# CESSProject/DeOSS

Hardware: AMD Instinct MI355X
Metric: device-resident GiB/s hashed to Merkle root; 1/2/4/8 MI355X scaling (higher is better)
Workload: dtype u32; 1 GPU; BASELINE configs[1]: 1 object of 8 GiB (8589934592 B) in 1 chunk-range shard(s) of 8 GiB, chunk 33554432 B (256 leaves); object_bytes=8589934592, chunk=33554432, leaves=256, parallelism=single GPU

## Files before the change

deoss_amd/csrc/merkle_kernels.hpp:

```cpp
#pragma once
#include "sha256_gfx950.hpp"

namespace dm {

constexpr int kBlock = 256;
constexpr int kLeafFuseMax = 8;
constexpr int kReduceTile = 512;

struct LeafArgs {
    const uint8_t* base;
    uint64_t pitch;
    uint64_t leaf_len;
    uint64_t last_len;
    const uint64_t* addrs;
    const uint64_t* lens;
    uint64_t nleaves;
    uint64_t byte_off;
    uint64_t byte_end;
    uint32_t* state;
    uint8_t* digests;
    uint8_t* level_out;
    uint32_t fuse_levels;
};

// ... 108 lines not shown
        compress(st, w);
    } else {
        compress(st, w);
#pragma unroll
        for (int k = 0; k < 14; k++) w[k] = 0;
        w[14] = (uint32_t)(bits >> 32);
        w[15] = (uint32_t)bits;
        compress(st, w);
    }
}

__device__ __forceinline__ uint32_t lds_reduce(uint32_t (*a)[8], uint32_t (*b)[8], uint32_t cnt,
                                               uint32_t levels, uint32_t (**res)[8]) {
    const uint32_t t = threadIdx.x;
    for (uint32_t l = 0; l < levels; l++) {
        const uint32_t next = (cnt + 1) >> 1;
        if (t < next) {
            uint32_t L[8], R[8], o[8];
            const uint32_t ri = (2 * t + 1 < cnt) ? 2 * t + 1 : cnt - 1;
#pragma unroll
            for (int k = 0; k < 8; k++) { L[k] = a[2 * t][k]; R[k] = a[ri][k]; }
            node_hash(L, R, o);
#pragma unroll
            for (int k = 0; k < 8; k++) b[t][k] = o[k];
        }
        __syncthreads();
        uint32_t (*tmp)[8] = a; a = b; b = tmp;
        cnt = next;
    }
    *res = a;
    return cnt;
}

struct LeafView {
    const uint8_t* p;
    uint64_t len;
    uint64_t have;
    uint64_t nb;
    bool fin;
    bool active;
};

template <bool TABLE>
__device__ __forceinline__ LeafView leaf_view(const LeafArgs& a, uint64_t i) {
    LeafView v{};
    v.active = i < a.nleaves;
    if (!v.active) {
        v.p = a.base;
        return v;
    }
    if constexpr (TABLE) {
        v.p = reinterpret_cast<const uint8_t*>(a.addrs[i]);
        v.len = a.lens[i];
    } else {
        v.p = a.base + i * a.pitch;
        v.len = (i + 1 == a.nleaves) ? a.last_len : a.leaf_len;
    }
    const uint64_t b0 = a.byte_off;
    const uint64_t end = v.len < a.byte_end ? v.len : a.byte_end;
    v.have = end > b0 ? end - b0 : 0;
    v.fin = (b0 < v.len && v.len <= a.byte_end) || (v.len == 0 && b0 == 0);
    v.nb = v.have / 64;
    return v;
}

__device__ __forceinline__ void load_or_init_state(const LeafArgs& a, uint64_t i, uint32_t (&st)[8]) {
    if (a.state != nullptr && a.byte_off != 0) {
#pragma unroll
        for (int k = 0; k < 8; k++) st[k] = a.state[i * 8 + k];
    } else {
        init_state(st);
    }
}

template <bool ALIGNED>
__device__ __forceinline__ void leaf_epilogue(const LeafArgs& a, uint64_t i, const LeafView& v, uint32_t (&st)[8]) {
    if (v.fin) {
        absorb_tail<ALIGNED>(st, v.p + 64 * v.nb, (uint32_t)(v.have - 64 * v.nb), v.len);
        if (a.digests != nullptr) store_digest(a.digests + 32 * i, st);
    } else if (a.state != nullptr && v.have != 0) {
#pragma unroll
        for (int k = 0; k < 8; k++) a.state[i * 8 + k] = st[k];
    }
}

__device__ __forceinline__ uint64_t wave_max_u64(uint64_t x) {
#pragma unroll
    for (int o = 32; o > 0; o >>= 1) {
        const uint64_t y = __shfl_xor(x, o, 64);
        x = y > x ? y : x;
    }
    return x;
}

template <bool TABLE, bool ALIGNED>
__global__ __launch_bounds__(kBlock) void leaf_kernel(LeafArgs a) {
    __shared__ uint32_t lds_a[kBlock][8];
    __shared__ uint32_t lds_b[kBlock / 2][8];
    const uint64_t i = (uint64_t)blockIdx.x * kBlock + threadIdx.x;
    const LeafView v = leaf_view<TABLE>(a, i);
    const bool active = v.active;
    uint32_t st[8];
    if (active) {
        load_or_init_state(a, i, st);
        absorb_blocks<ALIGNED>(st, v.p, v.nb);
        leaf_epilogue<ALIGNED>(a, i, v, st);
    }
    if (a.fuse_levels == 0) return;
    const uint64_t first = (uint64_t)blockIdx.x * kBlock;
    const uint32_t cnt = (uint32_t)((a.nleaves - first) < kBlock ? (a.nleaves - first) : kBlock);
    if (active) {
#pragma unroll
        for (int k = 0; k < 8; k++) lds_a[threadIdx.x][k] = st[k];
    }
    __syncthreads();
    uint32_t (*res)[8];
    const uint32_t out_cnt = lds_reduce(lds_a, lds_b, cnt, a.fuse_levels, &res);
    if (threadIdx.x < out_cnt) {
        uint32_t v[8];
#pragma unroll
        for (int k = 0; k < 8; k++) v[k] = res[threadIdx.x][k];
        const uint64_t o = (uint64_t)blockIdx.x * (kBlock >> a.fuse_levels) + threadIdx.x;
        store_digest(a.level_out + 32 * o, v);
    }
}

constexpr int kLatLeaves = 64;
constexpr int kLatThreads = 128;
constexpr int kLatRing = 2;
constexpr int kLatFuseMax = 6;

__device__ __forceinline__ void rounds_from_kw(uint32_t (&st)[8], const uint4 (*kw)[kLatLeaves], uint32_t lane) {
    uint32_t a = st[0], b = st[1], c = st[2], d = st[3], e = st[4], f = st[5], g = st[6], h = st[7];
    uint4 x = kw[0][lane], y = kw[1][lane];
#pragma unroll
    for (int q = 0; q < 16; q += 2) {
        uint4 nx = x, ny = y;
        if (q + 2 < 16) {
            nx = kw[q + 2][lane];
            ny = kw[q + 3][lane];
        }
        DM_SHA_ROUND(a, b, c, d, e, f, g, h, x.x);
        DM_SHA_ROUND(h, a, b, c, d, e, f, g, x.y);
        DM_SHA_ROUND(g, h, a, b, c, d, e, f, x.z);
        DM_SHA_ROUND(f, g, h, a, b, c, d, e, x.w);
        DM_SHA_ROUND(e, f, g, h, a, b, c, d, y.x);
        DM_SHA_ROUND(d, e, f, g, h, a, b, c, y.y);
        DM_SHA_ROUND(c, d, e, f, g, h, a, b, y.z);
        DM_SHA_ROUND(b, c, d, e, f, g, h, a, y.w);
        x = nx;
        y = ny;
    }
    st[0] += a; st[1] += b; st[2] += c; st[3] += d;
    st[4] += e; st[5] += f; st[6] += g; st[7] += h;
}

__device__ __forceinline__ void schedule_to_lds(uint32_t (&w)[16], uint4 (*kw)[kLatLeaves], uint32_t lane) {
#pragma unroll
    for (int q = 0; q < 16; q++) {
        uint32_t v[4];
#pragma unroll
        for (int j = 0; j < 4; j++) {
            const int t = 4 * q + j;
            uint32_t wt;
            if (t < 16) {
                wt = w[t];
// ... 109 lines not shown
    const uint64_t first = (uint64_t)blockIdx.x * kPairLeaves;
    const uint64_t i = first + c;
    const LeafView v = leaf_view<TABLE>(a, i);
    const uint64_t NB = wave_max_u64(v.nb);
    if (producer) {
        Blk cur;
        if (v.nb > 0 && !lane_b) cur = load_block<ALIGNED>(v.p);
        for (uint64_t b = 0; b < NB; b++) {
            if (b < v.nb) {
                uint32_t w[16];
                block_words(cur, w);
                if (b + 1 < v.nb && !lane_b) cur = load_block<ALIGNED>(v.p + 64 * (b + 1));
                uint4 (*kw)[kLatLeaves] = ring[b % kLatRing];
#pragma unroll
                for (int q = 0; q < 16; q++) {
                    uint32_t u[4];
#pragma unroll
                    for (int j = 0; j < 4; j++) {
                        const int t = 4 * q + j;
                        uint32_t wt;
                        if (t < 16) {
                            wt = w[t];
                        } else {
                            wt = ssig1(w[(t - 2) & 15]) + w[(t - 7) & 15] + ssig0(w[(t - 15) & 15]) + w[t & 15];
                            w[t & 15] = wt;
                        }
                        u[j] = lane_b ? 0u : kSha256K[t] + wt;
                    }
                    kw[q][lane] = make_uint4(u[0], u[1], u[2], u[3]);
                }
            }
            __syncthreads();
        }
        __syncthreads();
    } else {
        const uint32_t sh1 = lane_b ? 2 : 6, sh2 = lane_b ? 13 : 11, sh3 = lane_b ? 22 : 25;
        const uint32_t msk = lane_b ? 0u : ~0u;
        uint32_t st0[8];
        if (v.active) load_or_init_state(a, i, st0);
        else init_state(st0);
        uint32_t x[4];
#pragma unroll
        for (int k = 0; k < 4; k++) x[k] = lane_b ? st0[k] : st0[4 + k];
        __syncthreads();
        for (uint64_t b = 0; b < NB; b++) {
            if (b < v.nb) pair_rounds_from_kw(x, ring[b % kLatRing], lane, sh1, sh2, sh3, msk, lane_b);
            __syncthreads();
        }
        uint32_t st[8];
#pragma unroll
        for (int k = 0; k < 4; k++) {
            const uint32_t other = dpp_swap_pairs(x[k]);
            st[k] = lane_b ? x[k] : other;
            st[4 + k] = lane_b ? other : x[k];
        }
        if (v.active && !lane_b) {
            leaf_epilogue<ALIGNED>(a, i, v, st);
#pragma unroll
            for (int k = 0; k < 8; k++) lds_a[c][k] = st[k];
        }
    }
    if (a.fuse_levels == 0) return;
    __syncthreads();
    const uint32_t cnt = (uint32_t)((a.nleaves - first) < kPairLeaves ? (a.nleaves - first) : kPairLeaves);
    uint32_t (*res)[8];
    const uint32_t out_cnt = lds_reduce(lds_a, lds_b, cnt, a.fuse_levels, &res);
    if (threadIdx.x < out_cnt) {
        uint32_t o8[8];
#pragma unroll
        for (int k = 0; k < 8; k++) o8[k] = res[threadIdx.x][k];
        const uint64_t o = (uint64_t)blockIdx.x * (kPairLeaves >> a.fuse_levels) + threadIdx.x;
        store_digest(a.level_out + 32 * o, o8);
    }
}

constexpr int kQuadLeaves = 8;
constexpr int kQuadBlocks = 8;
constexpr int kQuadFuseMax = 3;
constexpr int kQuadRow = kQuadLeaves;
constexpr size_t kQuadLdsBytes = sizeof(uint4) * kLatRing * 16 * kQuadBlocks * kQuadRow + 4 * 8 * kQuadLeaves +
                                 4 * 8 * (kQuadLeaves / 2);
static_assert(4 * kQuadLdsBytes <= (160u << 10), "four compact K1Q workgroups must fit a CU's LDS");

#ifndef DM_QS_DEEP3
#define DM_QS_DEEP3 0
#endif
#if DM_QS_DEEP3
#define DM_QS_HEAD(X4, X5, X6)                                                                   \
    "v_alignbit_b32 %[r], %[" X4 "], %[" X4 "], %[sh]\n\t"                                      \
    "v_alignbit_b32 %[s], %[" X4 "], %[" X4 "], %[sh2]\n\t"                                     \
    "v_alignbit_b32 %[t], %[" X4 "], %[" X4 "], %[sh3]\n\t"                                     \
    "v_bitop3_b32 %[f], %[" X4 "], %[" X5 "], %[msk] bitop3:0x1e\n\t"                          \
    "v_bitop3_b32 %[f], %[f], %[" X6 "], %[" X5 "] bitop3:0xca\n\t"
#define DM_QS_SIGMA "v_bitop3_b32 %[s], %[r], %[s], %[t] bitop3:0x96\n\t"
#else
#define DM_QS_HEAD(X4, X5, X6)                                                                   \
    "v_alignbit_b32 %[r], %[" X4 "], %[" X4 "], %[sh]\n\t"                                      \
    "v_bitop3_b32 %[f], %[" X4 "], %[" X5 "], %[msk] bitop3:0x1e\n\t"                          \
    "v_bitop3_b32 %[f], %[f], %[" X6 "], %[" X5 "] bitop3:0xca\n\t"                             \
    "v_xor_b32_dpp %[s], %[r], %[r] quad_perm:[1,2,0,3] row_mask:0xf bank_mask:0xf\n\t"
#define DM_QS_SIGMA "v_xor_b32_dpp %[s], %[r], %[s] quad_perm:[2,0,1,3] row_mask:0xf bank_mask:0xf\n\t"
#endif
#define DM_QS_STEP_Q(X4, X5, X6, X7, H, HN, VN, QP)                                             \
    DM_QS_HEAD(X4, X5, X6)                                                                       \
    "v_sub_u32_dpp %[" X6 "], %[" VN "], %[" X6 "] quad_perm:" QP " row_mask:0xf bank_mask:0x3\n\t" \
    DM_QS_SIGMA                                                                                  \
    "v_sub_u32_dpp %[" HN "], %[" X4 "], %[" X6 "] row_ror:8 row_mask:0xf bank_mask:0xf\n\t"    \
    "v_add3_u32 %[" X7 "], %[s], %[f], %[" H "]\n\t"
#define DM_QS_STEP(X4, X5, X6, X7, H, HN, VN) DM_QS_STEP_Q(X4, X5, X6, X7, H, HN, VN, "[0,1,2,3]")
#define DM_QS_STEP_A(X4, X5, X6, X7, H, HN)                                                     \
    DM_QS_HEAD(X4, X5, X6)                                                                       \
    DM_QS_SIGMA                                                                                  \
    "v_sub_u32_dpp %[" HN "], %[" X4 "], %[" X6 "] row_ror:8 row_mask:0xf bank_mask:0xf\n\t"    \
    "v_add3_u32 %[" X7 "], %[s], %[f], %[" H "]\n\t"
#define DM_QS_STEP_END(X4, X5, X6, X7, H)                                                       \
    DM_QS_HEAD(X4, X5, X6)                                                                       \
    DM_QS_SIGMA                                                                                  \
    "v_add3_u32 %[" X7 "], %[s], %[f], %[" H "]\n\t"
#define DM_QS_STEPS4V(V0, V1, V2, V3)                                                          \
    DM_QS_STEP("a", "b", "c", "d", "h", "g", V0) DM_QS_STEP("d", "a", "b", "c", "g", "h", V1)   \
    DM_QS_STEP("c", "d", "a", "b", "h", "g", V2) DM_QS_STEP("b", "c", "d", "a", "g", "h", V3)
#define DM_QS_ALIGN ".p2align 3\n\t"
#define DM_QS_ALIGN_MIS ".p2align 3\n\t.if %[mis]\n\ts_nop 0\n\t.endif\n\t"
#define DM_QS_PROLOGUE(V) DM_QS_PROLOGUE_AT(V, DM_QS_ALIGN, "[0,1,2,3]")
#define DM_QS_PROLOGUE_AT(V, ALIGN, QP)                                                           \
    "s_nop 1\n\t" ALIGN                                                                          \
    "v_sub_u32_dpp %[d], %[" V "], %[d] quad_perm:" QP " row_mask:0xf bank_mask:0x3\n\t"         \
    "v_sub_u32_dpp %[h], %[b], %[d] row_ror:8 row_mask:0xf bank_mask:0xf\n\t"
#define DM_QS_RESTORE_A(P, X) "v_mov_b32_dpp %[" P "], %[" X "] quad_perm:[0,1,2,3] row_mask:0xf bank_mask:0xc\n\t"
#define DM_QS_GROUP0(V0, V1, V2, V3)                                                             \
    DM_QS_STEP("a", "b", "c", "d", "h", "g", V0) DM_QS_RESTORE_A("d", "x3")                      \
    DM_QS_STEP("d", "a", "b", "c", "g", "h", V1) DM_QS_RESTORE_A("c", "x2")                      \
    DM_QS_STEP("c", "d", "a", "b", "h", "g", V2) DM_QS_STEP("b", "c", "d", "a", "g", "h", V3)
#define DM_QS_FF(X, P, BANKS) "v_add_u32_dpp %[" X "], %[" P "], %[" X "] quad_perm:[0,1,2,3] row_mask:0xf bank_mask:" BANKS "\n\t"
#define DM_QS_TAIL(V0, V1, V2)                                                                   \
    DM_QS_STEP("a", "b", "c", "d", "h", "g", V0) DM_QS_STEP("d", "a", "b", "c", "g", "h", V1)   \
    DM_QS_STEP("c", "d", "a", "b", "h", "g", V2) DM_QS_STEP_A("b", "c", "d", "a", "g", "h")      \
    DM_QS_FF("x3", "d", "0x3") DM_QS_FF("x2", "c", "0x3") DM_QS_FF("x1", "b", "0x3")             \
    DM_QS_FF("x0", "a", "0x3")                                                                   \
    DM_QS_STEP_A("a", "b", "c", "d", "h", "g") DM_QS_STEP_END("d", "a", "b", "c", "g")           \
    DM_QS_FF("x0", "a", "0xc") DM_QS_FF("x1", "b", "0xc") DM_QS_FF("x3", "d", "0xc")             \
    DM_QS_FF("x2", "c", "0xc")
#define DM_QS_STEPS4Q(V0, Q0, V1, Q1, V2, Q2, V3, Q3)                                          \
    DM_QS_STEP_Q("a", "b", "c", "d", "h", "g", V0, Q0) DM_QS_STEP_Q("d", "a", "b", "c", "g", "h", V1, Q1) \
    DM_QS_STEP_Q("c", "d", "a", "b", "h", "g", V2, Q2) DM_QS_STEP_Q("b", "c", "d", "a", "g", "h", V3, Q3)
#define DM_QS_GROUP0Q(V0, Q0, V1, Q1, V2, Q2, V3, Q3)                                          \
    DM_QS_STEP_Q("a", "b", "c", "d", "h", "g", V0, Q0) DM_QS_RESTORE_A("d", "x3")              \
    DM_QS_STEP_Q("d", "a", "b", "c", "g", "h", V1, Q1) DM_QS_RESTORE_A("c", "x2")              \
    DM_QS_STEP_Q("c", "d", "a", "b", "h", "g", V2, Q2) DM_QS_STEP_Q("b", "c", "d", "a", "g", "h", V3, Q3)
#define DM_QS_TAILQ(V0, Q0, V1, Q1, V2, Q2)                                                     \
    DM_QS_STEP_Q("a", "b", "c", "d", "h", "g", V0, Q0) DM_QS_STEP_Q("d", "a", "b", "c", "g", "h", V1, Q1) \
    DM_QS_STEP_Q("c", "d", "a", "b", "h", "g", V2, Q2) DM_QS_STEP_A("b", "c", "d", "a", "g", "h") \
    DM_QS_FF("x3", "d", "0x3") DM_QS_FF("x2", "c", "0x3") DM_QS_FF("x1", "b", "0x3")             \
    DM_QS_FF("x0", "a", "0x3")                                                                   \
    DM_QS_STEP_A("a", "b", "c", "d", "h", "g") DM_QS_STEP_END("d", "a", "b", "c", "g")           \
    DM_QS_FF("x0", "a", "0xc") DM_QS_FF("x1", "b", "0xc") DM_QS_FF("x3", "d", "0xc")             \
    DM_QS_FF("x2", "c", "0xc")
#if DM_QS_DEEP3
#define DM_QS_XOUT , [t] "=&v"(t_)
#define DM_QS_XIN , [sh2] "v"(sh.y), [sh3] "v"(sh.z)
#else
#define DM_QS_XOUT
#define DM_QS_XIN
#endif
#define DM_QS_OUT                                                                                \
    : [a] "+v"(p0), [b] "+v"(p1), [c] "+v"(p2), [d] "+v"(p3), [h] "+v"(h), [g] "+v"(g),           \
      [x0] "+v"(x[0]), [x1] "+v"(x[1]), [x2] "+v"(x[2]), [x3] "+v"(x[3]), [r] "=&v"(r_),          \
      [f] "=&v"(f_), [s] "=&v"(s_) DM_QS_XOUT
#define DM_QS_OPS DM_QS_OUT : [sh] "v"(sh.x), [msk] "v"(msk), [v0] "v"(v0), [v1] "v"(v1), [v2] "v"(v2), [v3] "v"(v3) DM_QS_XIN

template <class KW>
__device__ __forceinline__ void quad_block_skewed(uint32_t (&x)[4], KW kw, uint3 sh, uint32_t msk) {
    uint32_t p0 = x[0], p1 = x[1], p2 = x[2], p3 = x[3], h = 0, g = 0, r_, f_, s_, t_;
    (void)t_;
    uint4 q = kw(0), nq = kw(1);
    {
        const uint32_t v0 = q.x, v1 = 0, v2 = 0, v3 = 0;
        asm volatile(DM_QS_PROLOGUE("v0") DM_QS_OPS);
    }
#pragma unroll
    for (int grp = 0; grp < 16; grp++) {
        const uint4 nnq = grp + 2 < 16 ? kw(grp + 2) : nq;
        const uint32_t v0 = q.y, v1 = q.z, v2 = q.w, v3 = nq.x;
        if (grp == 0) {
            asm volatile(DM_QS_ALIGN DM_QS_GROUP0("v0", "v1", "v2", "v3") DM_QS_OPS);
        } else if (grp < 15) {
            asm volatile(DM_QS_ALIGN DM_QS_STEPS4V("v0", "v1", "v2", "v3") DM_QS_OPS);
        } else {
            asm volatile(DM_QS_ALIGN DM_QS_TAIL("v0", "v1", "v2") DM_QS_OPS);
        }
        q = nq;
        nq = nnq;
    }
}

constexpr int kLgkmWait0 = 0xC07F;

template <bool MIS>
__device__ __forceinline__ void quad_block_regs(uint32_t (&x)[4], const uint4 (&K)[4], uint3 sh, uint32_t msk) {
    uint32_t p0 = x[0], p1 = x[1], p2 = x[2], p3 = x[3], h, g, r_, f_, s_, t_;
    (void)t_;
    asm volatile(DM_QS_PROLOGUE_AT("q00", DM_QS_ALIGN_MIS, "[0,0,0,0]")
                 DM_QS_GROUP0Q("q01", "[0,0,0,0]", "q02", "[0,0,0,0]", "q03", "[0,0,0,0]", "q00", "[1,1,1,1]")
                 DM_QS_STEPS4Q("q01", "[1,1,1,1]", "q02", "[1,1,1,1]", "q03", "[1,1,1,1]", "q00", "[2,2,2,2]")
                 DM_QS_STEPS4Q("q01", "[2,2,2,2]", "q02", "[2,2,2,2]", "q03", "[2,2,2,2]", "q00", "[3,3,3,3]")
                 DM_QS_STEPS4Q("q01", "[3,3,3,3]", "q02", "[3,3,3,3]", "q03", "[3,3,3,3]", "q10", "[0,0,0,0]")
                 DM_QS_STEPS4Q("q11", "[0,0,0,0]", "q12", "[0,0,0,0]", "q13", "[0,0,0,0]", "q10", "[1,1,1,1]")
                 DM_QS_STEPS4Q("q11", "[1,1,1,1]", "q12", "[1,1,1,1]", "q13", "[1,1,1,1]", "q10", "[2,2,2,2]")
                 DM_QS_STEPS4Q("q11", "[2,2,2,2]", "q12", "[2,2,2,2]", "q13", "[2,2,2,2]", "q10", "[3,3,3,3]")
                 DM_QS_STEPS4Q("q11", "[3,3,3,3]", "q12", "[3,3,3,3]", "q13", "[3,3,3,3]", "q20", "[0,0,0,0]")
                 DM_QS_STEPS4Q("q21", "[0,0,0,0]", "q22", "[0,0,0,0]", "q23", "[0,0,0,0]", "q20", "[1,1,1,1]")
                 DM_QS_STEPS4Q("q21", "[1,1,1,1]", "q22", "[1,1,1,1]", "q23", "[1,1,1,1]", "q20", "[2,2,2,2]")
                 DM_QS_STEPS4Q("q21", "[2,2,2,2]", "q22", "[2,2,2,2]", "q23", "[2,2,2,2]", "q20", "[3,3,3,3]")
                 DM_QS_STEPS4Q("q21", "[3,3,3,3]", "q22", "[3,3,3,3]", "q23", "[3,3,3,3]", "q30", "[0,0,0,0]")
                 DM_QS_STEPS4Q("q31", "[0,0,0,0]", "q32", "[0,0,0,0]", "q33", "[0,0,0,0]", "q30", "[1,1,1,1]")
                 DM_QS_STEPS4Q("q31", "[1,1,1,1]", "q32", "[1,1,1,1]", "q33", "[1,1,1,1]", "q30", "[2,2,2,2]")
                 DM_QS_STEPS4Q("q31", "[2,2,2,2]", "q32", "[2,2,2,2]", "q33", "[2,2,2,2]", "q30", "[3,3,3,3]")
                 DM_QS_TAILQ("q31", "[3,3,3,3]", "q32", "[3,3,3,3]", "q33", "[3,3,3,3]")
                 : [a] "+v"(p0), [b] "+v"(p1), [c] "+v"(p2), [d] "+v"(p3), [h] "=&v"(h), [g] "=&v"(g),
                   [x0] "+v"(x[0]), [x1] "+v"(x[1]), [x2] "+v"(x[2]), [x3] "+v"(x[3]), [r] "=&v"(r_),
                   [f] "=&v"(f_), [s] "=&v"(s_) DM_QS_XOUT
                 : [mis] "i"(MIS ? 1 : 0), [sh] "v"(sh.x), [msk] "v"(msk),
                   [q00] "v"(K[0].x), [q01] "v"(K[0].y), [q02] "v"(K[0].z), [q03] "v"(K[0].w),
                   [q10] "v"(K[1].x), [q11] "v"(K[1].y), [q12] "v"(K[1].z), [q13] "v"(K[1].w),
                   [q20] "v"(K[2].x), [q21] "v"(K[2].y), [q22] "v"(K[2].z), [q23] "v"(K[2].w),
                   [q30] "v"(K[3].x), [q31] "v"(K[3].y), [q32] "v"(K[3].z), [q33] "v"(K[3].w) DM_QS_XIN);
}

template <int G, int ROW, bool MIS>
__device__ __forceinline__ void quad_stage_regs(uint32_t (&x)[4], const uint4* kw, uint3 sh, uint32_t msk) {
    uint4 A[4], B[4];
#pragma unroll
    for (int t = 0; t < 4; t++) A[t] = kw[4 * t * G];
#pragma unroll
    for (int k = 0; k < kQuadBlocks; k += 2) {
        __builtin_amdgcn_s_waitcnt(kLgkmWait0);
#pragma unroll
        for (int t = 0; t < 4; t++) B[t] = kw[(k + 1) * ROW + 4 * t * G];
        quad_block_regs<MIS>(x, A, sh, msk);
        __builtin_amdgcn_s_waitcnt(kLgkmWait0);
        if (k + 2 < kQuadBlocks) {
#pragma unroll
            for (int t = 0; t < 4; t++) A[t] = kw[(k + 2) * ROW + 4 * t * G];
        }
        quad_block_regs<MIS>(x, B, sh, msk);
    }
}

template <bool TABLE, bool ALIGNED, bool COMPACT>
__global__ __launch_bounds__(kLatThreads) void leaf_kernel_quad(LeafArgs a) {
    constexpr int ROW = COMPACT ? kQuadRow : kQuadLeaves;
    constexpr int G = kQuadBlocks * ROW;
    __shared__ uint4 ring[COMPACT ? 1 : 2][kLatRing][16][G];
    __shared__ uint32_t lds_a[kQuadLeaves][8];
    __shared__ uint32_t lds_b[kQuadLeaves / 2][8];
    const uint32_t lane = threadIdx.x & 63;
    const bool producer = __builtin_amdgcn_readfirstlane(threadIdx.x) < 64;
    const uint32_t c = lane >> 3;
    const uint32_t j = lane & 7;
    const uint64_t first = (uint64_t)blockIdx.x * kQuadLeaves;
    const uint64_t i = first + c;
    const LeafView v = leaf_view<TABLE>(a, i);
    const uint64_t NB = wave_max_u64(v.nb);
    const uint64_t NI = (NB + kQuadBlocks - 1) / kQuadBlocks;
    if (producer) {
        Blk cur;
        if (j < v.nb) cur = load_block<ALIGNED>(v.p + 64 * j);
        for (uint64_t it = 0; it < NI; it++) {
            const uint64_t b = it * kQuadBlocks + j;
            if (b < v.nb) {
                uint32_t w[16];
                block_words(cur, w);
                if (b + kQuadBlocks < v.nb) cur = load_block<ALIGNED>(v.p + 64 * (b + kQuadBlocks));
                uint4* kw = &ring[0][it % kLatRing][0][j * ROW + c];
#pragma unroll
                for (int q = 0; q < 16; q++) {
                    uint32_t u[4];
#pragma unroll
                    for (int k = 0; k < 4; k++) {
                        const int t = 4 * q + k;
                        uint32_t wt;
                        if (t < 16) {
                            wt = w[t];
                        } else {
                            wt = ssig1(w[(t - 2) & 15]) + w[(t - 7) & 15] + ssig0(w[(t - 15) & 15]) + w[t & 15];
                            w[t & 15] = wt;
                        }
                        u[k] = 0u - (kSha256K[t] + wt);
                    }
                    kw[q * G] = make_uint4(u[0], u[1], u[2], u[3]);
                }
            }
            __syncthreads();
        }
        __syncthreads();
    } else {
        __builtin_amdgcn_s_setprio(1);
        const uint32_t cq = 2 * (lane >> 4) + ((lane >> 2) & 1);
        const bool role_a = (lane >> 3) & 1;
        const uint32_t p = lane & 3;
        const uint64_t iq = first + cq;
        const LeafView vq = leaf_view<TABLE>(a, iq);
#if DM_QS_DEEP3
        const uint3 sh = role_a ? make_uint3(2, 13, 22) : make_uint3(6, 11, 25);
#else
        const uint3 sh = make_uint3(role_a ? (p == 0 ? 2 : p == 1 ? 13 : 22) : (p == 0 ? 6 : p == 1 ? 11 : 25), 0, 0);
#endif
        const uint32_t msk = role_a ? 0u : ~0u;
        uint32_t st0[8];
        if (vq.active) load_or_init_state(a, iq, st0);
        else init_state(st0);
        uint32_t x[4];
#pragma unroll
        for (int k = 0; k < 4; k++) x[k] = role_a ? st0[(k + 2) & 3] : st0[4 + k];
        const uint4* col = &ring[0][0][0][cq];
        __syncthreads();
        uint32_t xf[4];
#pragma unroll
        for (int k = 0; k < 4; k++) xf[k] = x[k];
        auto partial = [&](uint64_t it) {
            const uint64_t b0 = it * kQuadBlocks;
            return __any(vq.active && vq.nb > b0 && vq.nb < b0 + kQuadBlocks);
        };
        for (uint64_t it = 0; it < NI;) {
            for (; it < NI && !partial(it); it++) {
                quad_stage_regs<G, ROW, COMPACT>(x, col + (it % kLatRing) * 16 * G + p * G, sh, msk);
                if (vq.nb > it * kQuadBlocks) {
#pragma unroll
                    for (int k = 0; k < 4; k++) xf[k] = x[k];
                }
                __syncthreads();
            }
            if (it == NI) break;
            const uint4* kw = col + (it % kLatRing) * 16 * G;
            const uint64_t b0 = it * kQuadBlocks;
            for (uint32_t k = 0; k < kQuadBlocks; k++) {
                const uint4* kb = kw + k * ROW;
                if (b0 + k < vq.nb)
                    quad_block_skewed(x, [kb](int g) { return kb[g * G]; }, sh, msk);
            }
            if (vq.nb > b0) {
#pragma unroll
                for (int k = 0; k < 4; k++) xf[k] = x[k];
            }
            __syncthreads();
            it++;
        }
        uint32_t st[8];
#pragma unroll
        for (int k = 0; k < 4; k++) {
            st[k] = __shfl(xf[(k + 2) & 3], (int)(lane + 8), 64);
            st[4 + k] = xf[k];
        }
        if (vq.active && !role_a && p == 0) {
            leaf_epilogue<ALIGNED>(a, iq, vq, st);
#pragma unroll
            for (int k = 0; k < 8; k++) lds_a[cq][k] = st[k];
        }
    }
    if (a.fuse_levels == 0) return;
    __syncthreads();
    const uint32_t cnt = (uint32_t)((a.nleaves - first) < kQuadLeaves ? (a.nleaves - first) : kQuadLeaves);
    uint32_t (*res)[8];
    const uint32_t out_cnt = lds_reduce(lds_a, lds_b, cnt, a.fuse_levels, &res);
    if (threadIdx.x < out_cnt) {
        uint32_t o8[8];
#pragma unroll
        for (int k = 0; k < 8; k++) o8[k] = res[threadIdx.x][k];
        const uint64_t o = (uint64_t)blockIdx.x * (kQuadLeaves >> a.fuse_levels) + threadIdx.x;
        store_digest(a.level_out + 32 * o, o8);
    }
}

__global__ __launch_bounds__(kLatThreads) void quad_shape_primer(int x) {
    extern __shared__ uint4 dyn[];
    if (x == 12345) dyn[threadIdx.x] = make_uint4(1, 1, 1, 1);
}

__global__ __launch_bounds__(kBlock) void reduce_kernel(const uint8_t* in, uint64_t m, uint32_t levels,
                                                         uint8_t* out) {
    __shared__ uint32_t lds_a[kBlock][8];
    __shared__ uint32_t lds_b[kBlock / 2][8];
    const uint64_t base = (uint64_t)blockIdx.x * kReduceTile;
    const uint32_t cnt = (uint32_t)((m - base) < kReduceTile ? (m - base) : kReduceTile);
    const uint32_t t = threadIdx.x;
    const uint32_t next = (cnt + 1) >> 1;
    if (t < next) {
        uint32_t L[8], R[8], o[8];
        const uint32_t ri = (2 * t + 1 < cnt) ? 2 * t + 1 : cnt - 1;
        load_digest(in + 32 * (base + 2 * t), L);
        load_digest(in + 32 * (base + ri), R);
        node_hash(L, R, o);
#pragma unroll
        for (int k = 0; k < 8; k++) lds_a[t][k] = o[k];
    }
    __syncthreads();
    uint32_t (*res)[8];
    const uint32_t out_cnt = lds_reduce(lds_a, lds_b, next, levels - 1, &res);
    if (t < out_cnt) {
        uint32_t v[8];
#pragma unroll
        for (int k = 0; k < 8; k++) v[k] = res[t][k];
        store_digest(out + 32 * ((uint64_t)blockIdx.x * (kReduceTile >> levels) + t), v);
    }
}

__global__ __launch_bounds__(kBlock) void batch_root_kernel(const uint8_t* leaves, const uint64_t* leaf_first,
                                                             const uint32_t* obj_ids, uint8_t* roots) {
    __shared__ uint32_t lds_a[kBlock][8];
    __shared__ uint32_t lds_b[kBlock / 2][8];
    const uint32_t o = obj_ids[blockIdx.x];
    const uint64_t base = leaf_first[o];
    const uint32_t cnt = (uint32_t)(leaf_first[o + 1] - base);
    const uint32_t t = threadIdx.x;
    const uint32_t next = (cnt + 1) >> 1;
    if (t < next) {
        uint32_t L[8], R[8], h[8];
        const uint32_t ri = (2 * t + 1 < cnt) ? 2 * t + 1 : cnt - 1;
        load_digest(leaves + 32 * (base + 2 * t), L);
        load_digest(leaves + 32 * (base + ri), R);
        node_hash(L, R, h);
#pragma unroll
// ... 68 lines not shown
```

deoss_amd/isa.py:

```python
from __future__ import annotations

import json
import os
import re
import subprocess
import tempfile

HERE = os.path.dirname(os.path.abspath(__file__))
COUNTS = os.path.join(HERE, "isa_counts.json")
SLOT_WEIGHTS = {"v_alignbit_b32": 2.0, "v_add3_u32": 2.0, "v_xad_u32": 2.0}
KERNELS = {
    "wide": ("_ZN2dm11leaf_kernelILb0ELb1EEEvNS_8LeafArgsE", (1, 0)),
    "latency": ("_ZN2dm15leaf_kernel_latILb0ELb1EEEvNS_8LeafArgsE", (1, 1)),
    "pair": ("_ZN2dm16leaf_kernel_pairILb0ELb1EEEvNS_8LeafArgsE", (2, 2)),
    "quad": ("_ZN2dm16leaf_kernel_quadILb0ELb1ELb0EEEvNS_8LeafArgsE", (8, 1)),
}
K1_SYMBOL = KERNELS["wide"][0]


def _function_body(asm: str, sym: str) -> list:
    lines = asm.splitlines()
    start = None
    for i, ln in enumerate(lines):
        if ln.startswith(sym + ":"):
            start = i
            break
    if start is None:
        raise ValueError(f"{sym} not found in assembly")
    body = []
    for ln in lines[start + 1:]:
        if ln.startswith(".Lfunc_end") or re.match(r"^\s*\.size\s+" + re.escape(sym), ln):
            break
        body.append(ln)
    return body


def _loops(body: list):
    labels, insts = {}, []
    skip = []
    for ln in body:
        s = ln.strip()
        m = re.match(r"^\.if\s+(\S+)", s)
        if m:
            skip.append(m.group(1) == "0")
            continue
        if s.startswith(".endif"):
            if skip:
                skip.pop()
            continue
        if any(skip):
            continue
        m = re.match(r"^(\.LBB[0-9_]+):", s)
        if m:
            labels[m.group(1)] = len(insts)
            continue
        if not s or s.startswith(";") or s.startswith("."):
            continue
        insts.append(s.split(";")[0].strip())
    for i, ins in enumerate(insts):
        m = re.match(r"^s_c?branch\w*\s+(\.LBB[0-9_]+)", ins)
        if m and m.group(1) in labels and labels[m.group(1)] <= i:
            yield insts[labels[m.group(1)]:i + 1]


def _summary(loop: list, per: int) -> dict:
    valu = [x for x in loop if x.startswith("v_")]
    hist = {}
    for x in valu:
        op = x.split()[0]
        hist[op] = hist.get(op, 0) + 1
    slots = sum(SLOT_WEIGHTS.get(x.split()[0], 1.0) for x in valu)
    return {"valu": round(len(valu) / per, 1), "valu_slots": round(slots / per, 1),
            "blocks_per_iteration": per, "salu": sum(1 for x in loop if x.startswith("s_")),
            "lds": sum(1 for x in loop if x.startswith("ds_")),
            "vmem": sum(1 for x in loop if x.startswith(("global_", "buffer_", "flat_"))),
            "total": len(loop), "valu_histogram": dict(sorted(hist.items(), key=lambda kv: -kv[1]))}


def _smallest(loops, pred):
    best = None
    for lp in loops:
        if pred(lp) and (best is None or len(lp) < len(best)):
            best = lp
    return best


def analyse(asm: str, sym: str = K1_SYMBOL) -> dict:
    loops = [l for l in _loops(_function_body(asm, sym))
             if sum(x.startswith("global_load_dwordx4") for x in l) >= 4]
    if not loops:
        raise ValueError("no block loop found")
    lp = max(loops, key=len)
    loads = sum(x.startswith("global_load_dwordx4") for x in lp)
    return _summary(lp, max(1, loads // 4))


def analyse_split(asm: str, sym: str) -> dict:
    loops = list(_loops(_function_body(asm, sym)))
    stage = _smallest(loops, lambda l: sum(x.startswith("v_add3_u32") for x in l) >= 8 * 66
                      and sum(x.startswith("ds_read_b128") for x in l) >= 32)
    if stage is not None:
        prod = _smallest(loops, lambda l: sum(x.startswith("ds_write_b128") for x in l) >= 16)
        if prod is None:
            raise ValueError(f"{sym}: producer loop not found")
        return {"consumer": _summary(stage, 8), "producer": _summary(prod, 1)}
    cons = _smallest(loops, lambda l: sum(x.startswith("ds_read_b128") for x in l) >= 16)
    prod = _smallest(loops, lambda l: sum(x.startswith("ds_write_b128") for x in l) >= 16)
    if cons is None or prod is None:
        raise ValueError(f"{sym}: consumer/producer loop not found")
    return {"consumer": _summary(cons, 1), "producer": _summary(prod, 1)}


def generate(write: bool = True) -> dict:
    from . import build as b
    with tempfile.TemporaryDirectory() as td:
        out = os.path.join(td, "lib.so")
        cmd = b.hipcc_cmd(out, extra=("-save-temps",))
        subprocess.run(cmd, check=True, cwd=td, capture_output=True)
        asm_files = [f for f in os.listdir(td) if f.endswith(".s") and "gfx950" in f]
        asm = open(os.path.join(td, asm_files[0])).read()
    res = {}
    for name, (sym, lanes) in KERNELS.items():
        if name == "wide":
            d = analyse(asm, sym)
            d["lane_slots_per_leaf_block"] = d["valu_slots"]
        else:
            d = analyse_split(asm, sym)
            d["lane_slots_per_leaf_block"] = (d["consumer"]["valu_slots"] * lanes[0] +
                                              d["producer"]["valu_slots"] * lanes[1])
            d["consumer_valu_per_block"] = d["consumer"]["valu"]
        d["kernel"] = sym
        d["lanes_per_leaf_block"] = {"consumer": lanes[0], "producer": lanes[1]}
        res[name] = d
    res["per"] = "one 64-byte block of one leaf"
    if write:
        with open(COUNTS, "w") as f:
            json.dump(res, f, indent=1)
    return res


def kernel_counts(kind: str = "wide"):
    try:
        with open(COUNTS) as f:
            d = json.load(f)[kind]
    except (OSError, KeyError, ValueError):
        return None, None
    ops = d["valu"] if kind == "wide" else d["consumer_valu_per_block"]
    return ops, d["lane_slots_per_leaf_block"]


def valu_per_block():
    return kernel_counts("wide")


def chain_instructions_per_block(kind: str):
    try:
        with open(COUNTS) as f:
            d = json.load(f)[kind]
    except (OSError, KeyError, ValueError):
        return None
    w = d if kind == "wide" else d.get("consumer", {})
    if "total" not in w or not w.get("blocks_per_iteration"):
        return None
    return w["total"] / w["blocks_per_iteration"]


if __name__ == "__main__":
    print(json.dumps(generate(), indent=1))
```

Measured before the change: 16.37 GiB/s.

## Chain quad SHA-256 blocks across a stage with fused feed-forward linking

Rewrites the per-stage quad-lane SHA-256 loop so the eight blocks of a stage are chained through a recursive template. Working state and h/g stay in registers between blocks, and each block's feed-forward and the next block's first rounds are fused into a link sequence. K-word loads move to a three-slot rotating register buffer. The wave loop now computes a uniform run length with a wave-min so that full-stage iterations skip the per-iteration partial check and the per-iteration finalize copy. It also removes the DEEP3 variant and applies misalignment padding to the skewed path, at the cost of more complex inline assembly and higher register pressure.

```diff
diff --git a/deoss_amd/csrc/merkle_kernels.hpp b/deoss_amd/csrc/merkle_kernels.hpp
--- a/deoss_amd/csrc/merkle_kernels.hpp
+++ b/deoss_amd/csrc/merkle_kernels.hpp
@@ -214,6 +214,20 @@
 #pragma unroll
         for (int k = 0; k < 8; k++) a.state[i * 8 + k] = st[k];
     }
+}
+
+__device__ __forceinline__ uint64_t wave_min_u64(uint64_t x) {
+#pragma unroll
+    for (int o = 32; o > 0; o >>= 1) {
+        const uint64_t y = __shfl_xor(x, o, 64);
+        x = y < x ? y : x;
+    }
+    return x;
+}
+
+__device__ __forceinline__ uint64_t uniform_u64(uint64_t x) {
+    return ((uint64_t)__builtin_amdgcn_readfirstlane((uint32_t)(x >> 32)) << 32) |
+           __builtin_amdgcn_readfirstlane((uint32_t)x);
 }
 
 __device__ __forceinline__ uint64_t wave_max_u64(uint64_t x) {
@@ -489,25 +503,12 @@
                                  4 * 8 * (kQuadLeaves / 2);
 static_assert(4 * kQuadLdsBytes <= (160u << 10), "four compact K1Q workgroups must fit a CU's LDS");
 
-#ifndef DM_QS_DEEP3
-#define DM_QS_DEEP3 0
-#endif
-#if DM_QS_DEEP3
-#define DM_QS_HEAD(X4, X5, X6)                                                                   \
-    "v_alignbit_b32 %[r], %[" X4 "], %[" X4 "], %[sh]\n\t"                                      \
-    "v_alignbit_b32 %[s], %[" X4 "], %[" X4 "], %[sh2]\n\t"                                     \
-    "v_alignbit_b32 %[t], %[" X4 "], %[" X4 "], %[sh3]\n\t"                                     \
-    "v_bitop3_b32 %[f], %[" X4 "], %[" X5 "], %[msk] bitop3:0x1e\n\t"                          \
-    "v_bitop3_b32 %[f], %[f], %[" X6 "], %[" X5 "] bitop3:0xca\n\t"
-#define DM_QS_SIGMA "v_bitop3_b32 %[s], %[r], %[s], %[t] bitop3:0x96\n\t"
-#else
 #define DM_QS_HEAD(X4, X5, X6)                                                                   \
     "v_alignbit_b32 %[r], %[" X4 "], %[" X4 "], %[sh]\n\t"                                      \
     "v_bitop3_b32 %[f], %[" X4 "], %[" X5 "], %[msk] bitop3:0x1e\n\t"                          \
     "v_bitop3_b32 %[f], %[f], %[" X6 "], %[" X5 "] bitop3:0xca\n\t"                             \
     "v_xor_b32_dpp %[s], %[r], %[r] quad_perm:[1,2,0,3] row_mask:0xf bank_mask:0xf\n\t"
 #define DM_QS_SIGMA "v_xor_b32_dpp %[s], %[r], %[s] quad_perm:[2,0,1,3] row_mask:0xf bank_mask:0xf\n\t"
-#endif
 #define DM_QS_STEP_Q(X4, X5, X6, X7, H, HN, VN, QP)                                             \
     DM_QS_HEAD(X4, X5, X6)                                                                       \
     "v_sub_u32_dpp %[" X6 "], %[" VN "], %[" X6 "] quad_perm:" QP " row_mask:0xf bank_mask:0x3\n\t" \
@@ -527,9 +528,8 @@
 #define DM_QS_STEPS4V(V0, V1, V2, V3)                                                          \
     DM_QS_STEP("a", "b", "c", "d", "h", "g", V0) DM_QS_STEP("d", "a", "b", "c", "g", "h", V1)   \
     DM_QS_STEP("c", "d", "a", "b", "h", "g", V2) DM_QS_STEP("b", "c", "d", "a", "g", "h", V3)
-#define DM_QS_ALIGN ".p2align 3\n\t"
 #define DM_QS_ALIGN_MIS ".p2align 3\n\t.if %[mis]\n\ts_nop 0\n\t.endif\n\t"
-#define DM_QS_PROLOGUE(V) DM_QS_PROLOGUE_AT(V, DM_QS_ALIGN, "[0,1,2,3]")
+#define DM_QS_PROLOGUE(V) DM_QS_PROLOGUE_AT(V, DM_QS_ALIGN_MIS, "[0,1,2,3]")
 #define DM_QS_PROLOGUE_AT(V, ALIGN, QP)                                                           \
     "s_nop 1\n\t" ALIGN                                                                          \
     "v_sub_u32_dpp %[d], %[" V "], %[d] quad_perm:" QP " row_mask:0xf bank_mask:0x3\n\t"         \
@@ -563,23 +563,15 @@
     DM_QS_STEP_A("a", "b", "c", "d", "h", "g") DM_QS_STEP_END("d", "a", "b", "c", "g")           \
     DM_QS_FF("x0", "a", "0xc") DM_QS_FF("x1", "b", "0xc") DM_QS_FF("x3", "d", "0xc")             \
     DM_QS_FF("x2", "c", "0xc")
-#if DM_QS_DEEP3
-#define DM_QS_XOUT , [t] "=&v"(t_)
-#define DM_QS_XIN , [sh2] "v"(sh.y), [sh3] "v"(sh.z)
-#else
-#define DM_QS_XOUT
-#define DM_QS_XIN
-#endif
 #define DM_QS_OUT                                                                                \
     : [a] "+v"(p0), [b] "+v"(p1), [c] "+v"(p2), [d] "+v"(p3), [h] "+v"(h), [g] "+v"(g),           \
       [x0] "+v"(x[0]), [x1] "+v"(x[1]), [x2] "+v"(x[2]), [x3] "+v"(x[3]), [r] "=&v"(r_),          \
-      [f] "=&v"(f_), [s] "=&v"(s_) DM_QS_XOUT
-#define DM_QS_OPS DM_QS_OUT : [sh] "v"(sh.x), [msk] "v"(msk), [v0] "v"(v0), [v1] "v"(v1), [v2] "v"(v2), [v3] "v"(v3) DM_QS_XIN
-
-template <class KW>
+      [f] "=&v"(f_), [s] "=&v"(s_)
+#define DM_QS_OPS DM_QS_OUT : [mis] "i"(MIS ? 1 : 0), [sh] "v"(sh.x), [msk] "v"(msk), [v0] "v"(v0), [v1] "v"(v1), [v2] "v"(v2), [v3] "v"(v3)
+
+template <bool MIS, class KW>
 __device__ __forceinline__ void quad_block_skewed(uint32_t (&x)[4], KW kw, uint3 sh, uint32_t msk) {
-    uint32_t p0 = x[0], p1 = x[1], p2 = x[2], p3 = x[3], h = 0, g = 0, r_, f_, s_, t_;
-    (void)t_;
+    uint32_t p0 = x[0], p1 = x[1], p2 = x[2], p3 = x[3], h = 0, g = 0, r_, f_, s_;
     uint4 q = kw(0), nq = kw(1);
     {
         const uint32_t v0 = q.x, v1 = 0, v2 = 0, v3 = 0;
@@ -590,11 +582,11 @@
         const uint4 nnq = grp + 2 < 16 ? kw(grp + 2) : nq;
         const uint32_t v0 = q.y, v1 = q.z, v2 = q.w, v3 = nq.x;
         if (grp == 0) {
-            asm volatile(DM_QS_ALIGN DM_QS_GROUP0("v0", "v1", "v2", "v3") DM_QS_OPS);
+            asm volatile(DM_QS_ALIGN_MIS DM_QS_GROUP0("v0", "v1", "v2", "v3") DM_QS_OPS);
         } else if (grp < 15) {
-            asm volatile(DM_QS_ALIGN DM_QS_STEPS4V("v0", "v1", "v2", "v3") DM_QS_OPS);
+            asm volatile(DM_QS_ALIGN_MIS DM_QS_STEPS4V("v0", "v1", "v2", "v3") DM_QS_OPS);
         } else {
-            asm volatile(DM_QS_ALIGN DM_QS_TAIL("v0", "v1", "v2") DM_QS_OPS);
+            asm volatile(DM_QS_ALIGN_MIS DM_QS_TAIL("v0", "v1", "v2") DM_QS_OPS);
         }
         q = nq;
         nq = nnq;
@@ -603,55 +595,102 @@
 
 constexpr int kLgkmWait0 = 0xC07F;
 
-template <bool MIS>
-__device__ __forceinline__ void quad_block_regs(uint32_t (&x)[4], const uint4 (&K)[4], uint3 sh, uint32_t msk) {
-    uint32_t p0 = x[0], p1 = x[1], p2 = x[2], p3 = x[3], h, g, r_, f_, s_, t_;
-    (void)t_;
-    asm volatile(DM_QS_PROLOGUE_AT("q00", DM_QS_ALIGN_MIS, "[0,0,0,0]")
-                 DM_QS_GROUP0Q("q01", "[0,0,0,0]", "q02", "[0,0,0,0]", "q03", "[0,0,0,0]", "q00", "[1,1,1,1]")
-                 DM_QS_STEPS4Q("q01", "[1,1,1,1]", "q02", "[1,1,1,1]", "q03", "[1,1,1,1]", "q00", "[2,2,2,2]")
-                 DM_QS_STEPS4Q("q01", "[2,2,2,2]", "q02", "[2,2,2,2]", "q03", "[2,2,2,2]", "q00", "[3,3,3,3]")
-                 DM_QS_STEPS4Q("q01", "[3,3,3,3]", "q02", "[3,3,3,3]", "q03", "[3,3,3,3]", "q10", "[0,0,0,0]")
-                 DM_QS_STEPS4Q("q11", "[0,0,0,0]", "q12", "[0,0,0,0]", "q13", "[0,0,0,0]", "q10", "[1,1,1,1]")
-                 DM_QS_STEPS4Q("q11", "[1,1,1,1]", "q12", "[1,1,1,1]", "q13", "[1,1,1,1]", "q10", "[2,2,2,2]")
-                 DM_QS_STEPS4Q("q11", "[2,2,2,2]", "q12", "[2,2,2,2]", "q13", "[2,2,2,2]", "q10", "[3,3,3,3]")
-                 DM_QS_STEPS4Q("q11", "[3,3,3,3]", "q12", "[3,3,3,3]", "q13", "[3,3,3,3]", "q20", "[0,0,0,0]")
-                 DM_QS_STEPS4Q("q21", "[0,0,0,0]", "q22", "[0,0,0,0]", "q23", "[0,0,0,0]", "q20", "[1,1,1,1]")
-                 DM_QS_STEPS4Q("q21", "[1,1,1,1]", "q22", "[1,1,1,1]", "q23", "[1,1,1,1]", "q20", "[2,2,2,2]")
-                 DM_QS_STEPS4Q("q21", "[2,2,2,2]", "q22", "[2,2,2,2]", "q23", "[2,2,2,2]", "q20", "[3,3,3,3]")
-                 DM_QS_STEPS4Q("q21", "[3,3,3,3]", "q22", "[3,3,3,3]", "q23", "[3,3,3,3]", "q30", "[0,0,0,0]")
-                 DM_QS_STEPS4Q("q31", "[0,0,0,0]", "q32", "[0,0,0,0]", "q33", "[0,0,0,0]", "q30", "[1,1,1,1]")
-                 DM_QS_STEPS4Q("q31", "[1,1,1,1]", "q32", "[1,1,1,1]", "q33", "[1,1,1,1]", "q30", "[2,2,2,2]")
-                 DM_QS_STEPS4Q("q31", "[2,2,2,2]", "q32", "[2,2,2,2]", "q33", "[2,2,2,2]", "q30", "[3,3,3,3]")
-                 DM_QS_TAILQ("q31", "[3,3,3,3]", "q32", "[3,3,3,3]", "q33", "[3,3,3,3]")
-                 : [a] "+v"(p0), [b] "+v"(p1), [c] "+v"(p2), [d] "+v"(p3), [h] "=&v"(h), [g] "=&v"(g),
-                   [x0] "+v"(x[0]), [x1] "+v"(x[1]), [x2] "+v"(x[2]), [x3] "+v"(x[3]), [r] "=&v"(r_),
-                   [f] "=&v"(f_), [s] "=&v"(s_) DM_QS_XOUT
-                 : [mis] "i"(MIS ? 1 : 0), [sh] "v"(sh.x), [msk] "v"(msk),
-                   [q00] "v"(K[0].x), [q01] "v"(K[0].y), [q02] "v"(K[0].z), [q03] "v"(K[0].w),
-                   [q10] "v"(K[1].x), [q11] "v"(K[1].y), [q12] "v"(K[1].z), [q13] "v"(K[1].w),
-                   [q20] "v"(K[2].x), [q21] "v"(K[2].y), [q22] "v"(K[2].z), [q23] "v"(K[2].w),
-                   [q30] "v"(K[3].x), [q31] "v"(K[3].y), [q32] "v"(K[3].z), [q33] "v"(K[3].w) DM_QS_XIN);
-}
-
+#define DM_QS_HNB(HN, A, B, BANKS) "v_sub_u32_dpp %[" HN "], %[" A "], %[" B "] row_ror:8 row_mask:0xf bank_mask:" BANKS "\n\t"
+#define DM_QS_ADDB(D, A, B, BANKS) "v_add_u32_dpp %[" D "], %[" A "], %[" B "] quad_perm:[0,1,2,3] row_mask:0xf bank_mask:" BANKS "\n\t"
+#define DM_QS_MOVB(D, S, BANKS) "v_mov_b32_dpp %[" D "], %[" S "] quad_perm:[0,1,2,3] row_mask:0xf bank_mask:" BANKS "\n\t"
+#define DM_QS_KWN(X6, S, N) "v_sub_u32_dpp %[" X6 "], %[" N "], %[" S "] quad_perm:[0,0,0,0] row_mask:0xf bank_mask:0x3\n\t"
+#define DM_QS_ADD3(X7, H) "v_add3_u32 %[" X7 "], %[s], %[f], %[" H "]\n\t"
+#define DM_QS_LINKQ(V0, Q0, V1, Q1, V2, Q2, N0, N1, N2)                                          \
+    DM_QS_STEP_Q("a", "b", "c", "d", "h", "g", V0, Q0) DM_QS_STEP_Q("d", "a", "b", "c", "g", "h", V1, Q1) \
+    DM_QS_STEP_Q("c", "d", "a", "b", "h", "g", V2, Q2)                                           \
+    DM_QS_ADDB("x1", "x1", "b", "0xc") DM_QS_ADDB("x3", "x3", "d", "0x3")                        \
+                                            \
+    DM_QS_HEAD("b", "c", "d") DM_QS_KWN("d", "x3", N0) DM_QS_SIGMA                               \
+    DM_QS_HNB("h", "x1", "d", "0x3") DM_QS_HNB("h", "b", "d", "0xc") DM_QS_ADD3("a", "g")        \
+    DM_QS_ADDB("b", "x1", "b", "0x3") DM_QS_ADDB("c", "x2", "c", "0x3")                          \
+    DM_QS_HNB("g", "a", "c", "0xc") DM_QS_ADDB("x0", "x0", "a", "0xc")                           \
+    DM_QS_ADDB("a", "a", "x0", "0x3") DM_QS_MOVB("x2", "c", "0x3")                               \
+                                                            \
+    DM_QS_HEAD("a", "b", "c") DM_QS_KWN("c", "c", N1) DM_QS_SIGMA                                \
+    DM_QS_HNB("g", "x0", "c", "0x3") DM_QS_ADD3("d", "h")                                        \
+    DM_QS_ADDB("x3", "x3", "d", "0xc") DM_QS_MOVB("x1", "b", "0x3") DM_QS_MOVB("x0", "a", "0x3") \
+                                           \
+    DM_QS_HEAD("d", "a", "b") DM_QS_KWN("b", "b", N2) DM_QS_SIGMA                                \
+    DM_QS_HNB("h", "x3", "b", "0x3") DM_QS_HNB("h", "d", "x1", "0xc") DM_QS_ADD3("c", "g")       \
+    DM_QS_ADDB("x2", "x2", "c", "0xc") DM_QS_MOVB("a", "x0", "0xc") DM_QS_MOVB("d", "x3", "0xc") \
+    DM_QS_MOVB("c", "x2", "0xc")
+#define DM_QS_BODYQ                                                                              \
+    DM_QS_STEPS4Q("q01", "[1,1,1,1]", "q02", "[1,1,1,1]", "q03", "[1,1,1,1]", "q00", "[2,2,2,2]") \
+    DM_QS_STEPS4Q("q01", "[2,2,2,2]", "q02", "[2,2,2,2]", "q03", "[2,2,2,2]", "q00", "[3,3,3,3]") \
+    DM_QS_STEPS4Q("q01", "[3,3,3,3]", "q02", "[3,3,3,3]", "q03", "[3,3,3,3]", "q10", "[0,0,0,0]") \
+    DM_QS_STEPS4Q("q11", "[0,0,0,0]", "q12", "[0,0,0,0]", "q13", "[0,0,0,0]", "q10", "[1,1,1,1]") \
+    DM_QS_STEPS4Q("q11", "[1,1,1,1]", "q12", "[1,1,1,1]", "q13", "[1,1,1,1]", "q10", "[2,2,2,2]") \
+    DM_QS_STEPS4Q("q11", "[2,2,2,2]", "q12", "[2,2,2,2]", "q13", "[2,2,2,2]", "q10", "[3,3,3,3]") \
+    DM_QS_STEPS4Q("q11", "[3,3,3,3]", "q12", "[3,3,3,3]", "q13", "[3,3,3,3]", "q20", "[0,0,0,0]") \
+    DM_QS_STEPS4Q("q21", "[0,0,0,0]", "q22", "[0,0,0,0]", "q23", "[0,0,0,0]", "q20", "[1,1,1,1]") \
+    DM_QS_STEPS4Q("q21", "[1,1,1,1]", "q22", "[1,1,1,1]", "q23", "[1,1,1,1]", "q20", "[2,2,2,2]") \
+    DM_QS_STEPS4Q("q21", "[2,2,2,2]", "q22", "[2,2,2,2]", "q23", "[2,2,2,2]", "q20", "[3,3,3,3]") \
+    DM_QS_STEPS4Q("q21", "[3,3,3,3]", "q22", "[3,3,3,3]", "q23", "[3,3,3,3]", "q30", "[0,0,0,0]") \
+    DM_QS_STEPS4Q("q31", "[0,0,0,0]", "q32", "[0,0,0,0]", "q33", "[0,0,0,0]", "q30", "[1,1,1,1]") \
+    DM_QS_STEPS4Q("q31", "[1,1,1,1]", "q32", "[1,1,1,1]", "q33", "[1,1,1,1]", "q30", "[2,2,2,2]") \
+    DM_QS_STEPS4Q("q31", "[2,2,2,2]", "q32", "[2,2,2,2]", "q33", "[2,2,2,2]", "q30", "[3,3,3,3]")
+#define DM_QS_FILLQ                                                                              \
+    DM_QS_PROLOGUE_AT("q00", DM_QS_ALIGN_MIS, "[0,0,0,0]")                                       \
+    DM_QS_GROUP0Q("q01", "[0,0,0,0]", "q02", "[0,0,0,0]", "q03", "[0,0,0,0]", "q00", "[1,1,1,1]")
+#define DM_QS_CONTQ                                                                              \
+    DM_QS_ALIGN_MIS                                                                              \
+    DM_QS_STEP_Q("c", "d", "a", "b", "h", "g", "q03", "[0,0,0,0]") DM_QS_STEP_Q("b", "c", "d", "a", "g", "h", "q00", "[1,1,1,1]")
+#define DM_QS_ENDLINKQ DM_QS_LINKQ("q31", "[3,3,3,3]", "q32", "[3,3,3,3]", "q33", "[3,3,3,3]", "n0", "n1", "n2")
+#define DM_QS_ENDTAILQ DM_QS_TAILQ("q31", "[3,3,3,3]", "q32", "[3,3,3,3]", "q33", "[3,3,3,3]")
+#define DM_QS_STATE [a] "+v"(P[0]), [b] "+v"(P[1]), [c] "+v"(P[2]), [d] "+v"(P[3]),              \
+                    [x0] "+v"(x[0]), [x1] "+v"(x[1]), [x2] "+v"(x[2]), [x3] "+v"(x[3]),           \
+                    [r] "=&v"(r_), [f] "=&v"(f_), [s] "=&v"(s_)
+#define DM_QS_KIN [mis] "i"(MIS ? 1 : 0), [sh] "v"(sh.x), [msk] "v"(msk),                        \
+                  [q00] "v"(K[0].x), [q01] "v"(K[0].y), [q02] "v"(K[0].z), [q03] "v"(K[0].w),     \
+                  [q10] "v"(K[1].x), [q11] "v"(K[1].y), [q12] "v"(K[1].z), [q13] "v"(K[1].w),     \
+                  [q20] "v"(K[2].x), [q21] "v"(K[2].y), [q22] "v"(K[2].z), [q23] "v"(K[2].w),     \
+                  [q30] "v"(K[3].x), [q31] "v"(K[3].y), [q32] "v"(K[3].z), [q33] "v"(K[3].w)
+
+template <bool MIS, int K8>
+__device__ __forceinline__ void quad_block_regs(uint32_t (&x)[4], uint32_t (&P)[4], uint32_t& h, uint32_t& g,
+                                                const uint4 (&K)[4], const uint4& N, uint3 sh, uint32_t msk) {
+    uint32_t r_, f_, s_;
+    if constexpr (K8 == 0) {
+        asm volatile(DM_QS_FILLQ DM_QS_BODYQ DM_QS_ENDLINKQ
+                     : DM_QS_STATE, [h] "=&v"(h), [g] "=&v"(g)
+                     : DM_QS_KIN, [n0] "v"(N.x), [n1] "v"(N.y), [n2] "v"(N.z));
+    } else if constexpr (K8 < kQuadBlocks - 1) {
+        asm volatile(DM_QS_CONTQ DM_QS_BODYQ DM_QS_ENDLINKQ
+                     : DM_QS_STATE, [h] "+v"(h), [g] "+v"(g)
+                     : DM_QS_KIN, [n0] "v"(N.x), [n1] "v"(N.y), [n2] "v"(N.z));
+    } else {
+        asm volatile(DM_QS_CONTQ DM_QS_BODYQ DM_QS_ENDTAILQ
+                     : DM_QS_STATE, [h] "+v"(h), [g] "+v"(g)
+                     : DM_QS_KIN);
+    }
+}
+
+template <int G, int ROW, bool MIS, int K8 = 0>
+__device__ __forceinline__ void quad_stage_blocks(uint32_t (&x)[4], uint32_t (&P)[4], uint32_t& h, uint32_t& g,
+                                                  uint4 (&S)[3][4], const uint4* kw, uint3 sh, uint32_t msk) {
+    __builtin_amdgcn_s_waitcnt(kLgkmWait0);
+    if constexpr (K8 + 2 < kQuadBlocks) {
+#pragma unroll
+        for (int t = 0; t < 4; t++) S[(K8 + 2) % 3][t] = kw[(K8 + 2) * ROW + 4 * t * G];
+    }
+    quad_block_regs<MIS, K8>(x, P, h, g, S[K8 % 3], S[(K8 + 1) % 3][0], sh, msk);
+    if constexpr (K8 + 1 < kQuadBlocks) quad_stage_blocks<G, ROW, MIS, K8 + 1>(x, P, h, g, S, kw, sh, msk);
+}
 template <int G, int ROW, bool MIS>
 __device__ __forceinline__ void quad_stage_regs(uint32_t (&x)[4], const uint4* kw, uint3 sh, uint32_t msk) {
-    uint4 A[4], B[4];
-#pragma unroll
-    for (int t = 0; t < 4; t++) A[t] = kw[4 * t * G];
-#pragma unroll
-    for (int k = 0; k < kQuadBlocks; k += 2) {
-        __builtin_amdgcn_s_waitcnt(kLgkmWait0);
-#pragma unroll
-        for (int t = 0; t < 4; t++) B[t] = kw[(k + 1) * ROW + 4 * t * G];
-        quad_block_regs<MIS>(x, A, sh, msk);
-        __builtin_amdgcn_s_waitcnt(kLgkmWait0);
-        if (k + 2 < kQuadBlocks) {
-#pragma unroll
-            for (int t = 0; t < 4; t++) A[t] = kw[(k + 2) * ROW + 4 * t * G];
-        }
-        quad_block_regs<MIS>(x, B, sh, msk);
-    }
+    uint4 S[3][4];
+    uint32_t P[4] = {x[0], x[1], x[2], x[3]}, h, g;
+#pragma unroll
+    for (int k = 0; k < 2; k++) {
+#pragma unroll
+        for (int t = 0; t < 4; t++) S[k][t] = kw[k * ROW + 4 * t * G];
+    }
+    quad_stage_blocks<G, ROW, MIS>(x, P, h, g, S, kw, sh, msk);
 }
 
 template <bool TABLE, bool ALIGNED, bool COMPACT>
@@ -708,11 +747,7 @@
         const uint32_t p = lane & 3;
         const uint64_t iq = first + cq;
         const LeafView vq = leaf_view<TABLE>(a, iq);
-#if DM_QS_DEEP3
-        const uint3 sh = role_a ? make_uint3(2, 13, 22) : make_uint3(6, 11, 25);
-#else
         const uint3 sh = make_uint3(role_a ? (p == 0 ? 2 : p == 1 ? 13 : 22) : (p == 0 ? 6 : p == 1 ? 11 : 25), 0, 0);
-#endif
         const uint32_t msk = role_a ? 0u : ~0u;
         uint32_t st0[8];
         if (vq.active) load_or_init_state(a, iq, st0);
@@ -725,26 +760,26 @@
         uint32_t xf[4];
 #pragma unroll
         for (int k = 0; k < 4; k++) xf[k] = x[k];
-        auto partial = [&](uint64_t it) {
-            const uint64_t b0 = it * kQuadBlocks;
-            return __any(vq.active && vq.nb > b0 && vq.nb < b0 + kQuadBlocks);
-        };
-        for (uint64_t it = 0; it < NI;) {
-            for (; it < NI && !partial(it); it++) {
+        const uint64_t NS = uniform_u64(NI);
+        for (uint64_t it = 0; it < NS;) {
+            const bool running = vq.active && vq.nb > it * kQuadBlocks;
+            const uint64_t end = uniform_u64(wave_min_u64(running ? vq.nb / kQuadBlocks : NS));
+            for (; it < end; it++) {
                 quad_stage_regs<G, ROW, COMPACT>(x, col + (it % kLatRing) * 16 * G + p * G, sh, msk);
-                if (vq.nb > it * kQuadBlocks) {
-#pragma unroll
-                    for (int k = 0; k < 4; k++) xf[k] = x[k];
-                }
                 __syncthreads();
             }
-            if (it == NI) break;
+            if (running) {
+#pragma unroll
+                for (int k = 0; k < 4; k++) xf[k] = x[k];
+            }
+            if (it == NS) break;
+            if (!__any(vq.active && vq.nb > it * kQuadBlocks && vq.nb < (it + 1) * kQuadBlocks)) continue;
             const uint4* kw = col + (it % kLatRing) * 16 * G;
             const uint64_t b0 = it * kQuadBlocks;
             for (uint32_t k = 0; k < kQuadBlocks; k++) {
                 const uint4* kb = kw + k * ROW;
                 if (b0 + k < vq.nb)
-                    quad_block_skewed(x, [kb](int g) { return kb[g * G]; }, sh, msk);
+                    quad_block_skewed<COMPACT>(x, [kb](int g) { return kb[g * G]; }, sh, msk);
             }
             if (vq.nb > b0) {
 #pragma unroll
diff --git a/deoss_amd/isa.py b/deoss_amd/isa.py
--- a/deoss_amd/isa.py
+++ b/deoss_amd/isa.py
@@ -97,7 +97,7 @@
 
 def analyse_split(asm: str, sym: str) -> dict:
     loops = list(_loops(_function_body(asm, sym)))
-    stage = _smallest(loops, lambda l: sum(x.startswith("v_add3_u32") for x in l) >= 8 * 66
+    stage = _smallest(loops, lambda l: sum(x.startswith("v_add3_u32") for x in l) >= 8 * 64 + 2
                       and sum(x.startswith("ds_read_b128") for x in l) >= 32)
     if stage is not None:
         prod = _smallest(loops, lambda l: sum(x.startswith("ds_write_b128") for x in l) >= 16)
```

New measurement: 16.77 GiB/s (median of 6 runs). 1.02x the previous value.
